# Gadersd/stable-diffusion-xl-burn

Hardware: NVIDIA H100
Metric: unet_sampler_steps_per_sec_1024x1024_bs1 (higher is better)
Workload: dtype f16

## Files before the change

### stable-diffusion-xl-burn_b200/csrc/attention.cu

```cuda
#include <stdlib.h>

#include "common.cuh"
#include "kernels.h"

namespace sdxl {

static constexpr int kTileBytes = 128 * 128;
static constexpr int kKvStages = 3;
static constexpr int kConsumerWarps = 8;
static constexpr int kAttnThreads = kConsumerWarps * 32 + 32;
static constexpr int kAttnSmem = 1024  + kTileBytes + 2 * kKvStages * kTileBytes + 256;

__device__ __forceinline__ float ex2_approx(float x) {
  float y;
  asm("ex2.approx.ftz.f32 %0, %1;" : "=f"(y) : "f"(x));
  return y;
}
__device__ __forceinline__ uint32_t pack_half2(float a, float b) {
  __half2 t = __floats2half2_rn(a, b);
  return *reinterpret_cast<uint32_t*>(&t);
}

__device__ __forceinline__ void attn_key_block(float (&o)[32], float (&m)[2], float (&l)[2], uint32_t q_addr, const uint8_t* sK,
                                               const uint8_t* sV, uint64_t* kv_full, uint64_t* kv_empty, int j, int kb, int S,
                                               float sl2e, int lane) {
  const int st = j % kKvStages;
  mbar_wait_nocall(&kv_full[st], (j / kKvStages) & 1);
  float s[64];
  wg_fence();
  const uint32_t k_addr = smem_u32(sK + st * kTileBytes);
#pragma unroll
  for (int k = 0; k < 4; ++k) wgmma_ss_n128(s, wg_desc_sw128(q_addr + 32 * k), wg_desc_sw128(k_addr + 32 * k), k);
  wg_commit();
  wg_wait<0>();
  if (kb * 128 + 128 > S) {
#pragma unroll
    for (int jj = 0; jj < 16; ++jj)
#pragma unroll
      for (int e = 0; e < 2; ++e)
        if (kb * 128 + 8 * jj + 2 * (lane & 3) + e >= S) { s[4 * jj + e] = -INFINITY; s[4 * jj + 2 + e] = -INFINITY; }
  }
  uint32_t pa[32];
#pragma unroll
  for (int h = 0; h < 2; ++h) {
    float mx = -INFINITY;
#pragma unroll
    for (int jj = 0; jj < 16; ++jj) mx = fmaxf(mx, fmaxf(s[4 * jj + 2 * h], s[4 * jj + 2 * h + 1]));
    mx = fmaxf(mx, __shfl_xor_sync(0xffffffffu, mx, 1));
    mx = fmaxf(mx, __shfl_xor_sync(0xffffffffu, mx, 2));
    const float m_new = fmaxf(m[h], mx);
    const float alpha = ex2_approx((m[h] - m_new) * sl2e);
    const float mb = m_new * sl2e;
    float sum = 0.f;
#pragma unroll
    for (int jj = 0; jj < 16; ++jj) {
      const float p0 = ex2_approx(fmaf(s[4 * jj + 2 * h], sl2e, -mb));
      const float p1 = ex2_approx(fmaf(s[4 * jj + 2 * h + 1], sl2e, -mb));
      sum += p0 + p1;
      pa[4 * (jj >> 1) + 2 * (jj & 1) + h] = pack_half2(p0, p1);
    }
    l[h] = l[h] * alpha + sum;
    m[h] = m_new;
#pragma unroll
    for (int jj = 0; jj < 8; ++jj) { o[4 * jj + 2 * h] *= alpha; o[4 * jj + 2 * h + 1] *= alpha; }
  }
  wg_fence();
  const uint32_t v_addr = smem_u32(sV + st * kTileBytes);
#pragma unroll
  for (int kk = 0; kk < 8; ++kk)
    wgmma_rs_n64_tb(o, *reinterpret_cast<const uint32_t(*)[4]>(pa + 4 * kk), wg_desc_sw128(v_addr + 2048 * kk));
  wg_commit();
  wg_wait<0>();
  if (lane == 0) mbar_arrive(&kv_empty[st]);
}

struct IpSrc {
  const CUtensorMap* tk;
  const CUtensorMap* tv;
  int S, k_col0, v_col0;
  const float* scale;
  const float* mask;
};
__device__ __forceinline__ IpSrc ip_source(const AttnParams& p, int k) {
  if (k == 0) return {&p.tmKip, &p.tmVip, p.S_ip, p.k_ip_col0, p.v_ip_col0, p.ip_scale, p.ip_mask};
  const AttnIpSource& s = p.ip_src[k - 1];
  return {&s.tm, &s.tm, s.S, s.k_col0, s.v_col0, s.scale, s.mask};
}

template <bool kIp>
__global__ void __launch_bounds__(kAttnThreads, 1) attention_kernel(const __grid_constant__ AttnParams p) {
  extern __shared__ uint8_t smem_raw[];
  uint8_t* smem = reinterpret_cast<uint8_t*>((reinterpret_cast<uintptr_t>(smem_raw) + 1023) & ~uintptr_t(1023));
  uint8_t* sQ = smem;
  uint8_t* sK = sQ + kTileBytes;
  uint8_t* sV = sK + kKvStages * kTileBytes;
  uint64_t* bars = reinterpret_cast<uint64_t*>(sV + kKvStages * kTileBytes);
  uint64_t* q_full = bars;
  uint64_t* kv_full = q_full + 1;
  uint64_t* kv_empty = kv_full + kKvStages;

  const int warp = threadIdx.x >> 5, lane = threadIdx.x & 31;
  const int nblk = (p.S + 127) / 128;
  const int nqt = (p.T + 127) / 128;
  const int qt = blockIdx.x % nqt, head = (blockIdx.x / nqt) % p.n_head, b = blockIdx.x / (nqt * p.n_head);

  if (threadIdx.x == 0) {
    tma_prefetch_desc(&p.tmQ);
    tma_prefetch_desc(&p.tmK);
    tma_prefetch_desc(&p.tmV);
    if constexpr (kIp) {
      tma_prefetch_desc(&p.tmKip);
      tma_prefetch_desc(&p.tmVip);
      for (int k = 1; k < p.n_src; ++k) tma_prefetch_desc(&p.ip_src[k - 1].tm);
    }
    mbar_init(q_full, 1);
    for (int i = 0; i < kKvStages; ++i) { mbar_init(&kv_full[i], 1); mbar_init(&kv_empty[i], kConsumerWarps); }
    fence_barrier_init();
  }
  __syncthreads();
  griddep_wait();
  griddep_launch_dependents();

  if (warp == kConsumerWarps) {
    if (lane != 0) return;
    mbar_expect_tx(q_full, kTileBytes);
    tma_load_3d(sQ, &p.tmQ, q_full, p.q_col0 + head * 64, qt * 128, b);
    for (int j = 0; j < nblk; ++j) {
      const int st = j % kKvStages;
      mbar_wait_nocall(&kv_empty[st], ((j / kKvStages) & 1) ^ 1);
      mbar_expect_tx(&kv_full[st], 2 * kTileBytes);
      tma_load_3d(sK + st * kTileBytes, &p.tmK, &kv_full[st], p.k_col0 + head * 64, j * 128, b);
      tma_load_3d(sV + st * kTileBytes, &p.tmV, &kv_full[st], p.v_col0 + head * 64, j * 128, b);
    }
    if constexpr (kIp) {
      int j = nblk;
      for (int k = 0; k < p.n_src; ++k) {
        const IpSrc s = ip_source(p, k);
        const int nb = (s.S + 127) / 128;
        for (int kb = 0; kb < nb; ++kb, ++j) {
          const int st = j % kKvStages;
          mbar_wait_nocall(&kv_empty[st], ((j / kKvStages) & 1) ^ 1);
          mbar_expect_tx(&kv_full[st], 2 * kTileBytes);
          tma_load_3d(sK + st * kTileBytes, s.tk, &kv_full[st], s.k_col0 + head * 64, kb * 128, b);
          tma_load_3d(sV + st * kTileBytes, s.tv, &kv_full[st], s.v_col0 + head * 64, kb * 128, b);
        }
      }
    }
    return;
  }

  const int wg = warp >> 2;
  const float sl2e = p.scale_log2e;
  const uint32_t q_addr = smem_u32(sQ) + (uint32_t)wg * (64 * 128);
  float o[32];
#pragma unroll
  for (int i = 0; i < 32; ++i) o[i] = 0.f;
  float m[2] = {-INFINITY, -INFINITY}, l[2] = {0.f, 0.f};
  mbar_wait_nocall(q_full, 0);
  for (int j = 0; j < nblk; ++j) {
    const int st = j % kKvStages;
    mbar_wait_nocall(&kv_full[st], (j / kKvStages) & 1);
    float s[64];
    wg_fence();
    const uint32_t k_addr = smem_u32(sK + st * kTileBytes);
#pragma unroll
    for (int k = 0; k < 4; ++k) wgmma_ss_n128(s, wg_desc_sw128(q_addr + 32 * k), wg_desc_sw128(k_addr + 32 * k), k);
    wg_commit();
    wg_wait<0>();
    if (j * 128 + 128 > p.S) {
#pragma unroll
      for (int jj = 0; jj < 16; ++jj)
#pragma unroll
        for (int e = 0; e < 2; ++e)
          if (j * 128 + 8 * jj + 2 * (lane & 3) + e >= p.S) { s[4 * jj + e] = -INFINITY; s[4 * jj + 2 + e] = -INFINITY; }
    }
    uint32_t pa[32];
#pragma unroll
    for (int h = 0; h < 2; ++h) {
      float mx = -INFINITY;
#pragma unroll
      for (int jj = 0; jj < 16; ++jj) mx = fmaxf(mx, fmaxf(s[4 * jj + 2 * h], s[4 * jj + 2 * h + 1]));
      mx = fmaxf(mx, __shfl_xor_sync(0xffffffffu, mx, 1));
      mx = fmaxf(mx, __shfl_xor_sync(0xffffffffu, mx, 2));
      const float m_new = fmaxf(m[h], mx);
      const float alpha = ex2_approx((m[h] - m_new) * sl2e);
      const float mb = m_new * sl2e;
      float sum = 0.f;
#pragma unroll
      for (int jj = 0; jj < 16; ++jj) {
        const float p0 = ex2_approx(fmaf(s[4 * jj + 2 * h], sl2e, -mb));
        const float p1 = ex2_approx(fmaf(s[4 * jj + 2 * h + 1], sl2e, -mb));
        sum += p0 + p1;
        pa[4 * (jj >> 1) + 2 * (jj & 1) + h] = pack_half2(p0, p1);
      }
      l[h] = l[h] * alpha + sum;
      m[h] = m_new;
#pragma unroll
      for (int jj = 0; jj < 8; ++jj) { o[4 * jj + 2 * h] *= alpha; o[4 * jj + 2 * h + 1] *= alpha; }
    }
    wg_fence();
    const uint32_t v_addr = smem_u32(sV + st * kTileBytes);
#pragma unroll
    for (int kk = 0; kk < 8; ++kk)
      wgmma_rs_n64_tb(o, *reinterpret_cast<const uint32_t(*)[4]>(pa + 4 * kk), wg_desc_sw128(v_addr + 2048 * kk));
    wg_commit();
    wg_wait<0>();
    if (lane == 0) mbar_arrive(&kv_empty[st]);
  }
  const int r = wg * 64 + (warp & 3) * 16 + (lane >> 2);
  if constexpr (kIp) {
    float acc[32];
#pragma unroll
    for (int h = 0; h < 2; ++h) {
      float lt = l[h];
      lt += __shfl_xor_sync(0xffffffffu, lt, 1);
      lt += __shfl_xor_sync(0xffffffffu, lt, 2);
      const float inv = 1.0f / lt;
#pragma unroll
      for (int jj = 0; jj < 8; ++jj) {
        acc[4 * jj + 2 * h] = o[4 * jj + 2 * h] * inv;
        acc[4 * jj + 2 * h + 1] = o[4 * jj + 2 * h + 1] * inv;
      }
    }
    int j = nblk;
    for (int k = 0; k < p.n_src; ++k) {
#pragma unroll
      for (int h = 0; h < 2; ++h) { m[h] = -INFINITY; l[h] = 0.f; }
#pragma unroll
      for (int i = 0; i < 32; ++i) o[i] = 0.f;
      const int S = ip_source(p, k).S;
      for (int kb = 0; kb * 128 < S; ++kb, ++j) attn_key_block(o, m, l, q_addr, sK, sV, kv_full, kv_empty, j, kb, S, sl2e, lane);
      const IpSrc s = ip_source(p, k);
      const float sk = *s.scale;
#pragma unroll
      for (int h = 0; h < 2; ++h) {
        float lt = l[h];
        lt += __shfl_xor_sync(0xffffffffu, lt, 1);
        lt += __shfl_xor_sync(0xffffffffu, lt, 2);
        const float inv = 1.0f / lt;
        const int t = qt * 128 + r + 8 * h;
        const float w = (s.mask && t < p.T) ? sk * s.mask[t] : sk;
#pragma unroll
        for (int jj = 0; jj < 8; ++jj) {
          acc[4 * jj + 2 * h] = fmaf(w, o[4 * jj + 2 * h] * inv, acc[4 * jj + 2 * h]);
          acc[4 * jj + 2 * h + 1] = fmaf(w, o[4 * jj + 2 * h + 1] * inv, acc[4 * jj + 2 * h + 1]);
        }
      }
    }
#pragma unroll
    for (int h = 0; h < 2; ++h) {
      const int t = qt * 128 + r + 8 * h;
      if (t < p.T) {
        __half* out = p.out + ((size_t)b * p.T + t) * p.ldo + head * 64 + 2 * (lane & 3);
#pragma unroll
        for (int jj = 0; jj < 8; ++jj)
          *reinterpret_cast<__half2*>(out + 8 * jj) = __floats2half2_rn(acc[4 * jj + 2 * h], acc[4 * jj + 2 * h + 1]);
      }
    }
  } else {
#pragma unroll
    for (int h = 0; h < 2; ++h) {
      float lt = l[h];
      lt += __shfl_xor_sync(0xffffffffu, lt, 1);
      lt += __shfl_xor_sync(0xffffffffu, lt, 2);
      const float inv = 1.0f / lt;
      const int t = qt * 128 + r + 8 * h;
      if (t < p.T) {
        __half* out = p.out + ((size_t)b * p.T + t) * p.ldo + head * 64 + 2 * (lane & 3);
#pragma unroll
        for (int jj = 0; jj < 8; ++jj)
          *reinterpret_cast<__half2*>(out + 8 * jj) = __floats2half2_rn(o[4 * jj + 2 * h] * inv, o[4 * jj + 2 * h + 1] * inv);
      }
    }
  }
}

__device__ __forceinline__ float cubic_w1(float x) { return ((-0.75f + 2.f) * x - (-0.75f + 3.f)) * x * x + 1.f; }
__device__ __forceinline__ float cubic_w2(float x) { return ((-0.75f * x - 5.f * -0.75f) * x + 8.f * -0.75f) * x - 4.f * -0.75f; }
__device__ __forceinline__ float cubic_1d(float x0, float x1, float x2, float x3, float t) {
  return x0 * cubic_w2(t + 1.f) + x1 * cubic_w1(t) + x2 * cubic_w1(1.f - t) + x3 * cubic_w2(2.f - t);
}
__global__ void ip_mask_resize_kernel(const float* __restrict__ mask, int H, int W, int mh, int mw, int T, float* __restrict__ out) {
  const int i = blockIdx.x * blockDim.x + threadIdx.x;
  if (i >= T) return;
  if (i >= mh * mw) { out[i] = 0.f; return; }
  const int oy = i / mw, ox = i % mw;
  const float ry = (float)H / mh * (oy + 0.5f) - 0.5f, rx = (float)W / mw * (ox + 0.5f) - 0.5f;
  const int iy = (int)floorf(ry), ix = (int)floorf(rx);
  const float ty = ry - iy, tx = rx - ix;
  float row[4];
#pragma unroll
  for (int k = 0; k < 4; ++k) {
    const float* m = mask + (size_t)min(max(iy - 1 + k, 0), H - 1) * W;
    row[k] = cubic_1d(m[min(max(ix - 1, 0), W - 1)], m[min(max(ix, 0), W - 1)], m[min(max(ix + 1, 0), W - 1)],
                      m[min(max(ix + 2, 0), W - 1)], tx);
  }
  out[i] = cubic_1d(row[0], row[1], row[2], row[3], ty);
}

int ip_mask_resize_launch(cudaStream_t st, const float* mask, int H, int W, int mh, int mw, int T, float* out) {
  if (H < 1 || W < 1 || mh < 1 || mw < 1 || T < 1) return 2002;
  ip_mask_resize_kernel<<<(T + 255) / 256, 256, 0, st>>>(mask, H, W, mh, mw, T, out);
  return (int)cudaGetLastError();
}

static bool g_attn_attr[2][64];
int attention_launch(cudaStream_t st, const AttnParams& p) {
  if (p.T < 1 || p.S < 1 || (p.ldo & 1)) return 2002;
  const bool ip = p.S_ip > 0;
  if (ip && (!p.ip_scale || p.n_src < 1 || p.n_src > ATTN_MAX_SRC)) return 2002;
  for (int k = 1; ip && k < p.n_src; ++k)
    if (p.ip_src[k - 1].S < 1 || !p.ip_src[k - 1].scale) return 2002;
  auto kernel = ip ? attention_kernel<true> : attention_kernel<false>;
  int r = smem_optin(kernel, kAttnSmem, g_attn_attr[ip]);
  if (r) return r;
  const long tiles = (long)p.B * p.n_head * ((p.T + 127) / 128);
  return launch_kernel(kernel, dim3((unsigned)tiles), dim3(kAttnThreads), (size_t)kAttnSmem, st, true, p);
}

}
```

### stable-diffusion-xl-burn_b200/csrc/kernels.h

```cpp
#pragma once
#include <cuda.h>
#include <cuda_fp16.h>
#include <cuda_runtime.h>
#include <stdint.h>

namespace sdxl {

bool pdl_enabled();
template <typename... KArgs, typename... Args>
inline int launch_kernel(void (*kernel)(KArgs...), dim3 grid, dim3 block, size_t smem, cudaStream_t st, bool pdl,
                         Args&&... args) {
  cudaLaunchConfig_t cfg{};
  cfg.gridDim = grid;
  cfg.blockDim = block;
  cfg.dynamicSmemBytes = smem;
  cfg.stream = st;
  cudaLaunchAttribute attr[1];
  attr[0].id = cudaLaunchAttributeProgrammaticStreamSerialization;
  attr[0].val.programmaticStreamSerializationAllowed = 1;
  cfg.attrs = attr;
  cfg.numAttrs = (pdl && pdl_enabled()) ? 1 : 0;
  return (int)cudaLaunchKernelEx(&cfg, kernel, static_cast<KArgs>(args)...);
}
template <typename... KArgs, typename... Args>
inline int launch_kernel_cluster(void (*kernel)(KArgs...), dim3 grid, dim3 block, size_t smem, cudaStream_t st, bool pdl,
                                 int cluster_size, Args&&... args) {
  cudaLaunchConfig_t cfg{};
  cfg.gridDim = grid;
  cfg.blockDim = block;
  cfg.dynamicSmemBytes = smem;
  cfg.stream = st;
  cudaLaunchAttribute attr[2];
  int n = 0;
  if (cluster_size > 1) {
    attr[n].id = cudaLaunchAttributeClusterDimension;
    attr[n].val.clusterDim.x = cluster_size;
    attr[n].val.clusterDim.y = 1;
    attr[n].val.clusterDim.z = 1;
    ++n;
  }
  if (pdl && pdl_enabled()) {
    attr[n].id = cudaLaunchAttributeProgrammaticStreamSerialization;
    attr[n].val.programmaticStreamSerializationAllowed = 1;
    ++n;
  }
  cfg.attrs = attr;
  cfg.numAttrs = n;
  return (int)cudaLaunchKernelEx(&cfg, kernel, static_cast<KArgs>(args)...);
}

template <typename K>
inline int smem_optin(K kernel, int bytes, bool (&done)[64]) {
  int dev = 0;
  cudaError_t e = cudaGetDevice(&dev);
  if (e != cudaSuccess) return (int)e;
  if (dev < 0 || dev >= 64) return 2001;
  if (!done[dev]) {
    e = cudaFuncSetAttribute(kernel, cudaFuncAttributeMaxDynamicSharedMemorySize, bytes);
    if (e != cudaSuccess) return (int)e;
    done[dev] = true;
  }
  return 0;
}

constexpr int IGEMM_MAX_SEG = 20;
struct IgemmSeg {
  int16_t map;
  int16_t dw, dh;
  int16_t db;
  int32_t nkb;
};
enum IgemmMode : int { IGEMM_LINEAR = 0, IGEMM_GEGLU = 1 };
struct alignas(64) IgemmParams {
  CUtensorMap tmA0, tmA1, tmB;
  IgemmSeg seg[IGEMM_MAX_SEG];
  int nseg;
  int Wt, Ht, Bt;
  int W, H, Bn;
  int tilesW, tilesH, tilesB, tilesN;
  int N;
  int BN;
  int nstages;
  int mode;
  void* out;
  int out_f32;
  int ldo;
  const float* bias;
  int bias_bstride;
  const float* res;
  int ldr;
  int opix_row, opix_w, opix_off;
};
int make_tmap_act(CUtensorMap* tm, const __half* base, int Bn, int H, int W, int C, int pitch, int Wt,
                  int Ht, int Bt);
int make_tmap_wgt(CUtensorMap* tm, const __half* base, int N, int K, int BN);
void igemm_pick_box(int W, int H, int* Wt, int* Ht, int* Bt);
struct IgemmOperands {
  const __half* a0; int a0Bn, a0H, a0W, a0C, a0pitch;
  const __half* a1; int a1Bn, a1H, a1W, a1C, a1pitch;
  const __half* w; int N, Ktot;
};
int igemm_configure(IgemmParams& p, const IgemmOperands& o, int outW, int outH, int outB, int mode, int geglu_bn);
int igemm_launch(cudaStream_t st, IgemmParams& p);
int igemm_pick_bn(int m_tiles, int N, int num_sms, bool geglu);

constexpr int ATTN_MAX_SRC = 8;
struct AttnIpSource {
  CUtensorMap tm;
  int S, k_col0, v_col0;
  const float* scale;
  const float* mask;
};
struct AttnParams {
  CUtensorMap tmQ, tmK, tmV;
  int T, S, n_head, B;
  int q_col0, k_col0, v_col0;
  __half* out;
  int ldo;
  float scale_log2e;
  CUtensorMap tmKip, tmVip;
  int S_ip;
  int k_ip_col0, v_ip_col0;
  const float* ip_scale;
  int n_src;
  const float* ip_mask;
  AttnIpSource ip_src[ATTN_MAX_SRC - 1];
};
int make_tmap_rows(CUtensorMap* tm, const __half* base, int rows_per_batch, int nbatch, int cols, int pitch);
int attention_launch(cudaStream_t st, const AttnParams& p);
int ip_mask_resize_launch(cudaStream_t st, const float* mask, int H, int W, int mh, int mw, int T, float* out);

struct GnParams {
  const float* x1; int C1;
  const float* x2; int C2;
  int B, HW, n_group;
  const float* gamma; const float* beta;
  float eps;
  int silu;
  __half* y;
  __half* raw;
  float* partial;
  int nchunk;
  __half* y_lo;
};
size_t gn_scratch_floats(int B, int n_group);
int gn_scratch_init(cudaStream_t st, float* scratch, int B, int n_group);
int gn_launch(cudaStream_t st, GnParams& p);
int layernorm_launch(cudaStream_t st, const float* x, const float* gamma, const float* beta, float eps,
                     int rows, int C, __half* y);

int gemv_launch(cudaStream_t st, const float* in, int in_bstride, int Bv, int K, const __half* W, int ldw,
                const float* bias, const float* add, int add_bstride, int N, int in_silu, int out_silu,
                float* out, int out_bstride);
int timestep_embedding_launch(cudaStream_t st, const int* t_dev, int nt, int dim, float max_period,
                              float* out);
int conv_in_launch(cudaStream_t st, const __half* x, int B, int Cin, int H, int W, const float* w,
                   const float* bias, int Cout, float* y);
int conv_in_launch_t(cudaStream_t st, const void* x, int x_f32, int Bx, int B, int Cin, int H, int W,
                     const float* w, const float* bias, int Cout, float* y, const float* add = nullptr, int n_add = 1);
int conv_in_cat_launch(cudaStream_t st, const void* x, int x_f32, int Bx, int B, int C1, const float* x2, int n2, int C2, int H, int W,
                       const float* w, const float* bias, int Cout, float* y, const float* add = nullptr, int n_add = 1);
int silu_f16_launch(cudaStream_t st, const float* x, int B, int H, int W, int C, int phase, __half* y);
int scale_weights_launch(cudaStream_t st, const __half* w, size_t nw, const float* b, int nb, float s, __half* wo, float* bo);
int upsample2x_launch(cudaStream_t st, const float* x, int B, int H, int W, int C, __half* y);
int phase_split_launch(cudaStream_t st, const float* x, int B, int H, int W, int C, __half* y);
int cast_f32_to_f16_launch(cudaStream_t st, const float* x, size_t n, __half* y);
int cast_f16_to_f32_launch(cudaStream_t st, const __half* x, size_t n, float* y);
int nhwc_to_nchw_f16_launch(cudaStream_t st, const float* x, int B, int HW, int C, int ldx, __half* y);
int nhwc_to_nchw_f32_launch(cudaStream_t st, const float* x, int B, int HW, int C, int ldx, float* y);
int cfg_ddim_launch(cudaStream_t st, const float* eps, int ld, int Bimg, int C, int HW, int use_cfg,
                    float guidance, float sqrt_a, float sqrt_1ma, float sqrt_ap, float sqrt_1map,
                    float* x, __half* x16);
int cfg_pag_ddim_launch(cudaStream_t st, const float* eps, int ld, int Bimg, int C, int HW, int use_cfg, float guidance, float p_t,
                        float sqrt_a, float sqrt_1ma, float sqrt_ap, float sqrt_1map, float* x);
int pag_identity_launch(cudaStream_t st, const __half* qkv, int C, long rows, __half* out);
int inpaint_blend_launch(cudaStream_t st, float* x, const float* ref, const float* noise,
                         const uint8_t* mask, size_t n_per_img_batch, int nfwd, float sqrt_a,
                         float sqrt_1ma, __half* x16);
int axpby_launch(cudaStream_t st, float* x, const float* noise, size_t n, float sa, float sb);
int randn_launch(cudaStream_t st, float* out, size_t n, uint64_t seed, uint64_t subseq);
int dup_latent_f16_launch(cudaStream_t st, const float* x, size_t n, int nfwd, __half* x16);

int softmax_rows_launch(cudaStream_t st, const float* S, size_t lds, int rows, int cols, float scale, __half* P,
                        size_t ldp);
int transpose_f16_launch(cudaStream_t st, const __half* x, size_t ldx, int rows, int cols, __half* y, size_t ldy);
int post_quant_launch(cudaStream_t st, const float* x, int B, int C, int HW, const float* w, const float* bias,
                      float inv_scale, float* y);
int image_u8_launch(cudaStream_t st, const float* x, long npix, int ldx, uint8_t* out);

int image_from_u8_launch(cudaStream_t st, const uint8_t* in, int B, long HW, float* out);
int quant_out_launch(cudaStream_t st, const float* x, int B, int Cz, int Cout, long HW, const float* w, const float* bias,
                     float scale, float* y);

int embed_tokens_launch(cudaStream_t st, const int* tokens, int rows, int T, int C, int n_vocab, const __half* tok_emb,
                        const __half* pos_emb, float* x, int* err);
int attention_small_launch(cudaStream_t st, const __half* q, int q_pitch, int q_col0, const __half* k, const __half* v,
                           int kv_pitch, int k_col0, int v_col0, int B, int T, int S, int n_head, const __half* mask,
                           int causal, __half* out, int ldo, int head_dim = 64);
int patchify_launch(cudaStream_t st, const float* pixels, int N, int S, int p, int Kpad, __half* y);
int vision_embed_ln_launch(cudaStream_t st, const float* patches, const __half* cls, const __half* pos, int N, int T, int C,
                           const float* gamma, const float* beta, float eps, float* x);
int mlp_act_launch(cudaStream_t st, const float* x, size_t n, int quick, __half* y);
int ln_gather_f32_launch(cudaStream_t st, const float* x, const int* idx, int B, int T, int C, const float* gamma,
                         const float* beta, float eps, float* y);
int perceiver_ln_launch(cudaStream_t st, const float* x, const float* lat, int n, int L, int Q, int C, const float* g1,
                        const float* b1, const float* g2, const float* b2, float eps, __half* kv, __half* q);

int pixel_unshuffle_launch(cudaStream_t st, const float* x, int n, int C, int H, int W, __half* y);
int relu_f16_launch(cudaStream_t st, const float* x, size_t n, __half* y);
int avg_pool2_f16_launch(cudaStream_t st, const float* x, int n, int H, int W, int C, __half* y);
int t2i_add_launch(cudaStream_t st, float* x, const float* F, long per_img, int B, int n_hint, const int* t, const int* t_min);

int transpose_linear_launch(cudaStream_t st, const __half* src, int K, int N, __half* dst, int Kpad,
                            int dst_row0, int geglu_bn);
int repack_conv_launch(cudaStream_t st, const __half* src, int O, int I, int KH, int KW, __half* dst,
                       int Ktot, int col0, int Ipad);
int repack_upconv_launch(cudaStream_t st, const __half* src, int O, int I, __half* dst, int Ipad);
int vec_add_f32_launch(cudaStream_t st, float* dst, const float* src, int n);
int bias_to_f32_launch(cudaStream_t st, const __half* src, int N, float* dst, int geglu_bn, int accumulate);

#define LORA_MAX_TERMS 16
struct LoraTerm { const __half* up; const __half* down; int r; float coef; };
struct LoraMergeParams {
  int N, Kd, taps;
  int nterm;
  LoraTerm term[LORA_MAX_TERMS];
  const void* src; void* dst; int f32;
  size_t ld; int row0, col0, Ipad, geglu_bn;
  float* delta_out;
};
int lora_merge_launch(cudaStream_t st, const LoraMergeParams& p);
int lora_upconv_merge_launch(cudaStream_t st, const __half* src, const float* delta, int O, int I, __half* dst, int Ipad);

}
```

### stable-diffusion-xl-burn_b200/csrc/testing.cu

```cuda
#include "kernels.h"

#define SDXL_TEST_API extern "C" __attribute__((visibility("default")))

using namespace sdxl;

SDXL_TEST_API int sdxl_test_igemm(void* stream, const void* a0, int a0Bn, int a0H, int a0W, int a0C, int a0pitch, const void* a1,
                                  int a1Bn, int a1H, int a1W, int a1C, int a1pitch, const void* w, int N, int Ktot, int outW,
                                  int outH, int outB, int mode, int geglu_bn, const int* segs, int nseg, void* out, int out_f32,
                                  int ldo, const float* bias, int bias_bstride, const float* res, int ldr, int opix_row,
                                  int opix_w, int opix_off) {
  if (nseg < 1 || nseg > IGEMM_MAX_SEG) return 5002;
  IgemmParams p{};
  p.nseg = nseg;
  for (int i = 0; i < nseg; ++i)
    p.seg[i] = {(int16_t)segs[5 * i], (int16_t)segs[5 * i + 1], (int16_t)segs[5 * i + 2], (int16_t)segs[5 * i + 3], segs[5 * i + 4]};
  p.out = out; p.out_f32 = out_f32; p.ldo = ldo;
  p.bias = bias; p.bias_bstride = bias_bstride;
  p.res = res; p.ldr = ldr;
  const IgemmOperands o{(const __half*)a0, a0Bn, a0H, a0W, a0C, a0pitch, (const __half*)a1, a1Bn, a1H, a1W, a1C, a1pitch,
                        (const __half*)w, N, Ktot};
  if (int r = igemm_configure(p, o, outW, outH, outB, mode, geglu_bn)) return r;
  if (opix_row) { p.opix_row = opix_row; p.opix_w = opix_w; p.opix_off = opix_off; }
  return igemm_launch((cudaStream_t)stream, p);
}

SDXL_TEST_API int sdxl_test_attention(void* stream, const void* q, int q_pitch, int q_col0, const void* kv, int kv_pitch, int k_col0,
                                      int v_col0, int B, int T, int S, int n_head, void* out, int ldo, const void* kip,
                                      int kip_pitch, int k_ip_col0, int v_ip_col0, int S_ip, const float* ip_scale) {
  AttnParams p{};
  p.T = T; p.S = S; p.n_head = n_head; p.B = B;
  p.q_col0 = q_col0; p.k_col0 = k_col0; p.v_col0 = v_col0;
  p.out = (__half*)out; p.ldo = ldo;
  p.scale_log2e = (float)(1.4426950408889634 / 8.0);
  int r = make_tmap_rows(&p.tmQ, (const __half*)q, T, B, q_pitch, q_pitch);
  if (!r) r = make_tmap_rows(&p.tmK, (const __half*)kv, S, B, kv_pitch, kv_pitch);
  if (r) return r;
  p.tmV = p.tmK;
  if (kip) {
    p.S_ip = S_ip; p.k_ip_col0 = k_ip_col0; p.v_ip_col0 = v_ip_col0; p.ip_scale = ip_scale; p.n_src = 1;
    if ((r = make_tmap_rows(&p.tmKip, (const __half*)kip, S_ip, B, kip_pitch, kip_pitch))) return r;
    p.tmVip = p.tmKip;
  }
  return attention_launch((cudaStream_t)stream, p);
}

SDXL_TEST_API int sdxl_test_attention_multi(void* stream, const void* q, int q_pitch, int q_col0, const void* kv, int kv_pitch, int k_col0,
                                            int v_col0, int B, int T, int S, int n_head, void* out, int ldo, int n_src,
                                            const void* const* src_kv, const int* src_info, const float* const* scales,
                                            const float* const* masks) {
  if (n_src < 1 || n_src > ATTN_MAX_SRC) return 5003;
  AttnParams p{};
  p.T = T; p.S = S; p.n_head = n_head; p.B = B;
  p.q_col0 = q_col0; p.k_col0 = k_col0; p.v_col0 = v_col0;
  p.out = (__half*)out; p.ldo = ldo;
  p.scale_log2e = (float)(1.4426950408889634 / 8.0);
  int r = make_tmap_rows(&p.tmQ, (const __half*)q, T, B, q_pitch, q_pitch);
  if (!r) r = make_tmap_rows(&p.tmK, (const __half*)kv, S, B, kv_pitch, kv_pitch);
  if (r) return r;
  p.tmV = p.tmK;
  p.n_src = n_src;
  for (int k = 0; k < n_src; ++k) {
    const int* f = src_info + 4 * k;
    CUtensorMap tm;
    if ((r = make_tmap_rows(&tm, (const __half*)src_kv[k], f[3], B, f[0], f[0]))) return r;
    if (k == 0) {
      p.tmKip = p.tmVip = tm;
      p.S_ip = f[3]; p.k_ip_col0 = f[1]; p.v_ip_col0 = f[2]; p.ip_scale = scales[0]; p.ip_mask = masks[0];
    } else {
      p.ip_src[k - 1] = {tm, f[3], f[1], f[2], scales[k], masks[k]};
    }
  }
  return attention_launch((cudaStream_t)stream, p);
}

SDXL_TEST_API int sdxl_test_ip_mask_resize(void* stream, const float* mask, int H, int W, int mh, int mw, int T, float* out) {
  return ip_mask_resize_launch((cudaStream_t)stream, mask, H, W, mh, mw, T, out);
}

SDXL_TEST_API int sdxl_test_attention_small(void* stream, const void* q, int q_pitch, int q_col0, const void* k, const void* v,
                                            int kv_pitch, int k_col0, int v_col0, int B, int T, int S, int n_head, const void* mask,
                                            int causal, void* out, int ldo, int head_dim) {
  return attention_small_launch((cudaStream_t)stream, (const __half*)q, q_pitch, q_col0, (const __half*)k, (const __half*)v, kv_pitch,
                                k_col0, v_col0, B, T, S, n_head, (const __half*)mask, causal, (__half*)out, ldo, head_dim);
}

SDXL_TEST_API int sdxl_test_perceiver_ln(void* stream, const float* x, const float* lat, int n, int L, int Q, int C, const float* g1,
                                         const float* b1, const float* g2, const float* b2, float eps, void* kv, void* q) {
  return perceiver_ln_launch((cudaStream_t)stream, x, lat, n, L, Q, C, g1, b1, g2, b2, eps, (__half*)kv, (__half*)q);
}

SDXL_TEST_API size_t sdxl_test_gn_scratch_floats(int B, int n_group) { return gn_scratch_floats(B, n_group); }
SDXL_TEST_API int sdxl_test_gn_scratch_init(void* stream, float* scratch, int B, int n_group) {
  return gn_scratch_init((cudaStream_t)stream, scratch, B, n_group);
}
SDXL_TEST_API int sdxl_test_gn(void* stream, const float* x1, int C1, const float* x2, int C2, int B, int HW, int n_group,
                               const float* gamma, const float* beta, float eps, int silu, void* y, void* raw, void* y_lo,
                               float* scratch) {
  GnParams p{x1, C1, x2, C2, B, HW, n_group, gamma, beta, eps, silu, (__half*)y, (__half*)raw, scratch, 0, (__half*)y_lo};
  return gn_launch((cudaStream_t)stream, p);
}

SDXL_TEST_API int sdxl_test_gemv(void* stream, const float* in, int in_bstride, int Bv, int K, const void* W, int ldw,
                                 const float* bias, const float* add, int add_bstride, int N, int in_silu, int out_silu, float* out,
                                 int out_bstride) {
  return gemv_launch((cudaStream_t)stream, in, in_bstride, Bv, K, (const __half*)W, ldw, bias, add, add_bstride, N, in_silu, out_silu,
                     out, out_bstride);
}

SDXL_TEST_API int sdxl_test_conv_in(void* stream, const void* x, int x_f32, int Bx, int B, int Cin, int H, int W, const float* w,
                                    const float* bias, int Cout, float* y, const float* add, int n_add) {
  return conv_in_launch_t((cudaStream_t)stream, x, x_f32, Bx, B, Cin, H, W, w, bias, Cout, y, add, n_add);
}
SDXL_TEST_API int sdxl_test_conv_in_cat(void* stream, const void* x, int x_f32, int Bx, int B, int C1, const float* x2, int n2, int C2,
                                        int H, int W, const float* w, const float* bias, int Cout, float* y) {
  return conv_in_cat_launch((cudaStream_t)stream, x, x_f32, Bx, B, C1, x2, n2, C2, H, W, w, bias, Cout, y);
}

SDXL_TEST_API int sdxl_test_pag_identity(void* stream, const void* qkv, int C, long rows, void* out) {
  return pag_identity_launch((cudaStream_t)stream, (const __half*)qkv, C, rows, (__half*)out);
}
SDXL_TEST_API int sdxl_test_cfg_pag_ddim(void* stream, const float* eps, int ld, int Bimg, int C, int HW, int use_cfg, float guidance,
                                         float p_t, float sqrt_a, float sqrt_1ma, float sqrt_ap, float sqrt_1map, float* x) {
  return cfg_pag_ddim_launch((cudaStream_t)stream, eps, ld, Bimg, C, HW, use_cfg, guidance, p_t, sqrt_a, sqrt_1ma, sqrt_ap, sqrt_1map, x);
}

SDXL_TEST_API int sdxl_test_repack_upconv(void* stream, const void* src, int O, int I, void* dst, int Ipad) {
  return repack_upconv_launch((cudaStream_t)stream, (const __half*)src, O, I, (__half*)dst, Ipad);
}
SDXL_TEST_API int sdxl_test_repack_conv(void* stream, const void* src, int O, int I, int KH, int KW, void* dst, int Ktot, int col0,
                                        int Ipad) {
  return repack_conv_launch((cudaStream_t)stream, (const __half*)src, O, I, KH, KW, (__half*)dst, Ktot, col0, Ipad);
}
SDXL_TEST_API int sdxl_test_transpose_linear(void* stream, const void* src, int K, int N, void* dst, int Kpad, int dst_row0,
                                             int geglu_bn) {
  return transpose_linear_launch((cudaStream_t)stream, (const __half*)src, K, N, (__half*)dst, Kpad, dst_row0, geglu_bn);
}
SDXL_TEST_API int sdxl_test_bias_to_f32(void* stream, const void* src, int N, float* dst, int geglu_bn, int accumulate) {
  return bias_to_f32_launch((cudaStream_t)stream, (const __half*)src, N, dst, geglu_bn, accumulate);
}

SDXL_TEST_API int sdxl_test_lora_merge(void* stream, int N, int Kd, int taps, int nterm, const void* const* up, const void* const* down,
                                       const int* r, const float* coef, const void* src, void* dst, int f32, size_t ld, int row0,
                                       int col0, int Ipad, int geglu_bn, float* delta_out) {
  if (nterm < 1 || nterm > LORA_MAX_TERMS) return 1;
  LoraMergeParams p{};
  p.N = N; p.Kd = Kd; p.taps = taps; p.nterm = nterm;
  for (int i = 0; i < nterm; ++i) p.term[i] = {(const __half*)up[i], (const __half*)down[i], r[i], coef[i]};
  p.src = src; p.dst = dst; p.f32 = f32;
  p.ld = ld; p.row0 = row0; p.col0 = col0; p.Ipad = Ipad; p.geglu_bn = geglu_bn;
  p.delta_out = delta_out;
  return lora_merge_launch((cudaStream_t)stream, p);
}
SDXL_TEST_API int sdxl_test_lora_upconv_merge(void* stream, const void* src, const float* delta, int O, int I, void* dst, int Ipad) {
  return lora_upconv_merge_launch((cudaStream_t)stream, (const __half*)src, delta, O, I, (__half*)dst, Ipad);
}
```

### stable-diffusion-xl-burn_b200/sdxl_b200/_testing.py

```python
from __future__ import annotations

import ctypes as C
import os
from typing import Optional, Sequence

import torch

from ._lib import SdxlError, SdxlLibraryMissing

HERE = os.path.dirname(os.path.abspath(__file__))
LIB_PATH = os.path.join(HERE, "libsdxl_b200_testing.so")

P, I, F = C.c_void_p, C.c_int, C.c_float
PROTOTYPES = {
    "sdxl_test_igemm": (I, [P, P, I, I, I, I, I, P, I, I, I, I, I, P, I, I, I, I, I, I, I, P, I, P, I, I, P, I, P, I, I, I, I]),
    "sdxl_test_attention": (I, [P, P, I, I, P, I, I, I, I, I, I, I, P, I, P, I, I, I, I, P]),
    "sdxl_test_attention_multi": (I, [P, P, I, I, P, I, I, I, I, I, I, I, P, I, I, P, P, P, P]),
    "sdxl_test_ip_mask_resize": (I, [P, P, I, I, I, I, I, P]),
    "sdxl_test_attention_small": (I, [P, P, I, I, P, P, I, I, I, I, I, I, I, P, I, P, I, I]),
    "sdxl_test_perceiver_ln": (I, [P, P, P, I, I, I, I, P, P, P, P, F, P, P]),
    "sdxl_test_gn_scratch_floats": (C.c_size_t, [I, I]),
    "sdxl_test_gn_scratch_init": (I, [P, P, I, I]),
    "sdxl_test_gn": (I, [P, P, I, P, I, I, I, I, P, P, F, I, P, P, P, P]),
    "sdxl_test_gemv": (I, [P, P, I, I, I, P, I, P, P, I, I, I, I, P, I]),
    "sdxl_test_conv_in": (I, [P, P, I, I, I, I, I, I, P, P, I, P, P, I]),
    "sdxl_test_conv_in_cat": (I, [P, P, I, I, I, I, P, I, I, I, I, P, P, I, P]),
    "sdxl_test_pag_identity": (I, [P, P, I, C.c_long, P]),
    "sdxl_test_cfg_pag_ddim": (I, [P, P, I, I, I, I, I, F, F, F, F, F, F, P]),
    "sdxl_test_repack_upconv": (I, [P, P, I, I, P, I]),
    "sdxl_test_repack_conv": (I, [P, P, I, I, I, I, P, I, I, I]),
    "sdxl_test_transpose_linear": (I, [P, P, I, I, P, I, I, I]),
    "sdxl_test_bias_to_f32": (I, [P, P, I, P, I, I]),
    "sdxl_test_lora_merge": (I, [P, I, I, I, I, P, P, P, P, P, P, I, C.c_size_t, I, I, I, I, P]),
    "sdxl_test_lora_upconv_merge": (I, [P, P, P, I, I, P, I]),
}
_lib = None


def load() -> C.CDLL:
    global _lib
    if _lib is None:
        if not os.path.exists(LIB_PATH):
            raise SdxlLibraryMissing(f"{LIB_PATH} not found: build it with `python stable-diffusion-xl-burn_b200/build.py`")
        lib = C.CDLL(LIB_PATH)
        for name, (res, args) in PROTOTYPES.items():
            fn = getattr(lib, name)
            fn.restype = res
            fn.argtypes = args
        _lib = lib
    return _lib


def _p(t: Optional[torch.Tensor]):
    if t is None:
        return None
    assert t.is_cuda and t.is_contiguous(), "kernel operands are contiguous CUDA tensors"
    return t.data_ptr()


def _call(name: str, *args) -> None:
    lib = load()
    rc = getattr(lib, name)(torch.cuda.current_stream().cuda_stream, *args)
    if rc != 0:
        raise SdxlError(f"{name} failed ({rc})")


def igemm(a0: torch.Tensor, a0_shape: Sequence[int], w: torch.Tensor, N: int, Ktot: int, out_whb: Sequence[int],
          segs: Sequence[Sequence[int]], out: torch.Tensor, ldo: int, *, a1: Optional[torch.Tensor] = None,
          a1_shape: Sequence[int] = (0, 0, 0, 0), bias: Optional[torch.Tensor] = None, bias_bstride: int = 0,
          res: Optional[torch.Tensor] = None, ldr: int = 0, mode: int = 0, geglu_bn: int = 0,
          opix: Optional[Sequence[int]] = None) -> None:
    seg = (C.c_int * (5 * len(segs)))(*[int(v) for s in segs for v in s])
    o = opix or (0, 0, 0)
    _call("sdxl_test_igemm", _p(a0), *a0_shape, a0_shape[3], _p(a1), *a1_shape, a1_shape[3], _p(w), N, Ktot, *out_whb, mode,
          geglu_bn, seg, len(segs), _p(out), int(out.dtype == torch.float32), ldo, _p(bias), bias_bstride, _p(res), ldr, *o)


def attention(q: torch.Tensor, q_pitch: int, q_col0: int, kv: torch.Tensor, kv_pitch: int, k_col0: int, v_col0: int,
              B: int, T: int, S: int, n_head: int, out: torch.Tensor, ldo: int, kip: Optional[torch.Tensor] = None,
              kip_pitch: int = 0, k_ip_col0: int = 0, v_ip_col0: int = 0, S_ip: int = 0,
              ip_scale: Optional[torch.Tensor] = None) -> None:
    _call("sdxl_test_attention", _p(q), q_pitch, q_col0, _p(kv), kv_pitch, k_col0, v_col0, B, T, S, n_head, _p(out), ldo,
          _p(kip), kip_pitch, k_ip_col0, v_ip_col0, S_ip, _p(ip_scale))


def attention_multi(q: torch.Tensor, q_pitch: int, q_col0: int, kv: torch.Tensor, kv_pitch: int, k_col0: int, v_col0: int,
                    B: int, T: int, S: int, n_head: int, out: torch.Tensor, ldo: int, sources: Sequence[tuple]) -> None:
    n = len(sources)
    kvs = (C.c_void_p * n)(*[_p(s[0]) for s in sources])
    info = (C.c_int * (4 * n))(*[int(v) for s in sources for v in (s[1], s[2], s[3], s[4])])
    scales = (C.c_void_p * n)(*[_p(s[5]) for s in sources])
    masks = (C.c_void_p * n)(*[_p(s[6]) for s in sources])
    _call("sdxl_test_attention_multi", _p(q), q_pitch, q_col0, _p(kv), kv_pitch, k_col0, v_col0, B, T, S, n_head, _p(out), ldo, n,
          kvs, info, scales, masks)


def ip_mask_resize(mask: torch.Tensor, mh: int, mw: int, T: int) -> torch.Tensor:
    out = torch.empty(T, device=mask.device, dtype=torch.float32)
    _call("sdxl_test_ip_mask_resize", _p(mask), mask.shape[0], mask.shape[1], mh, mw, T, _p(out))
    return out


def attention_small(q, q_pitch, q_col0, k, v, kv_pitch, k_col0, v_col0, B, T, S, n_head, mask, causal, out, ldo,
                    head_dim) -> None:
    _call("sdxl_test_attention_small", _p(q), q_pitch, q_col0, _p(k), _p(v), kv_pitch, k_col0, v_col0, B, T, S, n_head,
          _p(mask), int(causal), _p(out), ldo, head_dim)


def perceiver_ln(x, lat, n, L, Q, C, g1, b1, g2, b2, eps, kv, q) -> None:
    _call("sdxl_test_perceiver_ln", _p(x), _p(lat), n, L, Q, C, _p(g1), _p(b1), _p(g2), _p(b2), eps, _p(kv), _p(q))


def gn_scratch(B: int, n_group: int) -> torch.Tensor:
    s = torch.empty(load().sdxl_test_gn_scratch_floats(B, n_group), dtype=torch.float32, device="cuda")
    _call("sdxl_test_gn_scratch_init", _p(s), B, n_group)
    return s


def group_norm(x1, x2, B, HW, n_group, gamma, beta, eps, silu, y, raw, y_lo, scratch) -> None:
    C1 = x1.shape[-1]
    C2 = 0 if x2 is None else x2.shape[-1]
    _call("sdxl_test_gn", _p(x1), C1, _p(x2), C2, B, HW, n_group, _p(gamma), _p(beta), eps, int(silu), _p(y), _p(raw),
          _p(y_lo), _p(scratch))


def gemv(inp, in_bstride, Bv, K, W, ldw, bias, add, add_bstride, N, in_silu, out_silu, out, out_bstride) -> None:
    _call("sdxl_test_gemv", _p(inp), in_bstride, Bv, K, _p(W), ldw, _p(bias), _p(add), add_bstride, N, int(in_silu),
          int(out_silu), _p(out), out_bstride)


def conv_in(x, Bx, B, Cin, H, W, w, bias, Cout, y, add=None, n_add=1) -> None:
    _call("sdxl_test_conv_in", _p(x), int(x.dtype == torch.float32), Bx, B, Cin, H, W, _p(w), _p(bias), Cout, _p(y), _p(add),
          n_add)


def conv_in_cat(x, Bx, B, C1, x2, n2, C2, H, W, w, bias, Cout, y) -> None:
    _call("sdxl_test_conv_in_cat", _p(x), int(x.dtype == torch.float32), Bx, B, C1, _p(x2), n2, C2, H, W, _p(w), _p(bias), Cout, _p(y))


def pag_identity(qkv: torch.Tensor, C: int, rows: int, out: torch.Tensor) -> None:
    _call("sdxl_test_pag_identity", _p(qkv), C, rows, _p(out))


def cfg_pag_ddim(eps, ld, Bimg, C, HW, use_cfg, guidance, p_t, sqrt_a, sqrt_1ma, sqrt_ap, sqrt_1map, x) -> None:
    _call("sdxl_test_cfg_pag_ddim", _p(eps), ld, Bimg, C, HW, int(use_cfg), guidance, p_t, sqrt_a, sqrt_1ma, sqrt_ap, sqrt_1map, _p(x))


def repack_upconv(src, O, I, dst, Ipad) -> None:
    _call("sdxl_test_repack_upconv", _p(src), O, I, _p(dst), Ipad)


def repack_conv(src, O, I, KH, KW, dst, Ktot, col0, Ipad) -> None:
    _call("sdxl_test_repack_conv", _p(src), O, I, KH, KW, _p(dst), Ktot, col0, Ipad)


def transpose_linear(src, K, N, dst, Kpad, dst_row0=0, geglu_bn=0) -> None:
    _call("sdxl_test_transpose_linear", _p(src), K, N, _p(dst), Kpad, dst_row0, geglu_bn)


def bias_to_f32(src, N, dst, geglu_bn=0, accumulate=False) -> None:
    _call("sdxl_test_bias_to_f32", _p(src), N, _p(dst), geglu_bn, int(accumulate))


def lora_merge(N, Kd, taps, terms, src, dst, ld, row0=0, col0=0, Ipad=0, geglu_bn=0, delta_out=None) -> None:
    n = len(terms)
    ups = (C.c_void_p * n)(*[_p(u) for u, _, _ in terms])
    downs = (C.c_void_p * n)(*[_p(d) for _, d, _ in terms])
    rs = (C.c_int * n)(*[u.shape[1] for u, _, _ in terms])
    coefs = (C.c_float * n)(*[float(c) for _, _, c in terms])
    _call("sdxl_test_lora_merge", N, Kd, taps, n, ups, downs, rs, coefs, _p(src), _p(dst), int(dst.dtype == torch.float32), ld,
          row0, col0, Ipad, geglu_bn, _p(delta_out))


def lora_upconv_merge(src, delta, O, I, dst, Ipad) -> None:
    _call("sdxl_test_lora_upconv_merge", _p(src), _p(delta), O, I, _p(dst), Ipad)
```

Measured before the change: 27.65.

## Overlap next QK wgmma with PV in attention and skip unneeded rescale

Splits the attention key block into a QK issue step and a softmax/PV step, then issues the next block's QK wgmma before waiting on the current PV wgmma. This lets the tensor-core work of consecutive blocks overlap. It also skips rescaling the output accumulator when no row maximum grew in the warp. A polynomial exp2 emulation is added to offload work from the MUFU unit, but its column fraction is set to zero, so only the test kernel uses it for now. The s register array is now live across iterations, which raises register pressure.

```diff
diff --git a/stable-diffusion-xl-burn_b200/csrc/attention.cu b/stable-diffusion-xl-burn_b200/csrc/attention.cu
--- a/stable-diffusion-xl-burn_b200/csrc/attention.cu
+++ b/stable-diffusion-xl-burn_b200/csrc/attention.cu
@@ -16,22 +16,38 @@
   asm("ex2.approx.ftz.f32 %0, %1;" : "=f"(y) : "f"(x));
   return y;
 }
+__device__ __forceinline__ float ex2_poly(float x) {
+  x = fmaxf(x, -127.f);
+  const float t = x + 12582912.f;
+  const float f = x - (t - 12582912.f);
+  float p = fmaf(9.58323106e-3f, f, 5.59063852e-2f);
+  p = fmaf(p, f, 2.40240902e-1f);
+  p = fmaf(p, f, 6.93124235e-1f);
+  p = fmaf(p, f, 1.f);
+  return __int_as_float(__float_as_int(p) + (__float_as_int(t) << 23));
+}
+static constexpr int kPolyExp2 = 0;
+__device__ constexpr bool poly_col(int jj) { return jj * (kPolyExp2 / 4) / 16 != (jj + 1) * (kPolyExp2 / 4) / 16; }
 __device__ __forceinline__ uint32_t pack_half2(float a, float b) {
   __half2 t = __floats2half2_rn(a, b);
   return *reinterpret_cast<uint32_t*>(&t);
 }
 
-__device__ __forceinline__ void attn_key_block(float (&o)[32], float (&m)[2], float (&l)[2], uint32_t q_addr, const uint8_t* sK,
-                                               const uint8_t* sV, uint64_t* kv_full, uint64_t* kv_empty, int j, int kb, int S,
-                                               float sl2e, int lane) {
+__device__ __forceinline__ void attn_qk(float (&s)[64], uint32_t q_addr, const uint8_t* sK, uint64_t* kv_full, int j) {
   const int st = j % kKvStages;
   mbar_wait_nocall(&kv_full[st], (j / kKvStages) & 1);
-  float s[64];
   wg_fence();
   const uint32_t k_addr = smem_u32(sK + st * kTileBytes);
 #pragma unroll
   for (int k = 0; k < 4; ++k) wgmma_ss_n128(s, wg_desc_sw128(q_addr + 32 * k), wg_desc_sw128(k_addr + 32 * k), k);
   wg_commit();
+}
+
+template <bool kNext>
+__device__ __forceinline__ void attn_key_block(float (&s)[64], float (&o)[32], float (&m)[2], float (&l)[2], uint32_t q_addr,
+                                               const uint8_t* sK, const uint8_t* sV, uint64_t* kv_full, uint64_t* kv_empty, int j,
+                                               int kb, int S, float sl2e, int lane) {
+  const int st = j % kKvStages;
   wg_wait<0>();
   if (kb * 128 + 128 > S) {
 #pragma unroll
@@ -40,7 +56,7 @@
       for (int e = 0; e < 2; ++e)
         if (kb * 128 + 8 * jj + 2 * (lane & 3) + e >= S) { s[4 * jj + e] = -INFINITY; s[4 * jj + 2 + e] = -INFINITY; }
   }
-  uint32_t pa[32];
+  float m_new[2];
 #pragma unroll
   for (int h = 0; h < 2; ++h) {
     float mx = -INFINITY;
@@ -48,21 +64,31 @@
     for (int jj = 0; jj < 16; ++jj) mx = fmaxf(mx, fmaxf(s[4 * jj + 2 * h], s[4 * jj + 2 * h + 1]));
     mx = fmaxf(mx, __shfl_xor_sync(0xffffffffu, mx, 1));
     mx = fmaxf(mx, __shfl_xor_sync(0xffffffffu, mx, 2));
-    const float m_new = fmaxf(m[h], mx);
-    const float alpha = ex2_approx((m[h] - m_new) * sl2e);
-    const float mb = m_new * sl2e;
+    m_new[h] = fmaxf(m[h], mx);
+  }
+  const bool grown = __any_sync(0xffffffffu, m_new[0] != m[0] || m_new[1] != m[1]);
+  uint32_t pa[32];
+#pragma unroll
+  for (int h = 0; h < 2; ++h) {
+    const float mb = m_new[h] * sl2e;
     float sum = 0.f;
 #pragma unroll
     for (int jj = 0; jj < 16; ++jj) {
-      const float p0 = ex2_approx(fmaf(s[4 * jj + 2 * h], sl2e, -mb));
-      const float p1 = ex2_approx(fmaf(s[4 * jj + 2 * h + 1], sl2e, -mb));
+      const float x0 = fmaf(s[4 * jj + 2 * h], sl2e, -mb), x1 = fmaf(s[4 * jj + 2 * h + 1], sl2e, -mb);
+      const float p0 = poly_col(jj) ? ex2_poly(x0) : ex2_approx(x0);
+      const float p1 = poly_col(jj) ? ex2_poly(x1) : ex2_approx(x1);
       sum += p0 + p1;
       pa[4 * (jj >> 1) + 2 * (jj & 1) + h] = pack_half2(p0, p1);
     }
-    l[h] = l[h] * alpha + sum;
-    m[h] = m_new;
-#pragma unroll
-    for (int jj = 0; jj < 8; ++jj) { o[4 * jj + 2 * h] *= alpha; o[4 * jj + 2 * h + 1] *= alpha; }
+    if (grown) {
+      const float alpha = ex2_approx((m[h] - m_new[h]) * sl2e);
+      l[h] = fmaf(l[h], alpha, sum);
+#pragma unroll
+      for (int jj = 0; jj < 8; ++jj) { o[4 * jj + 2 * h] *= alpha; o[4 * jj + 2 * h + 1] *= alpha; }
+    } else {
+      l[h] += sum;
+    }
+    m[h] = m_new[h];
   }
   wg_fence();
   const uint32_t v_addr = smem_u32(sV + st * kTileBytes);
@@ -70,7 +96,12 @@
   for (int kk = 0; kk < 8; ++kk)
     wgmma_rs_n64_tb(o, *reinterpret_cast<const uint32_t(*)[4]>(pa + 4 * kk), wg_desc_sw128(v_addr + 2048 * kk));
   wg_commit();
-  wg_wait<0>();
+  if constexpr (kNext) {
+    attn_qk(s, q_addr, sK, kv_full, j + 1);
+    wg_wait<1>();
+  } else {
+    wg_wait<0>();
+  }
   if (lane == 0) mbar_arrive(&kv_empty[st]);
 }
 
@@ -157,56 +188,10 @@
   for (int i = 0; i < 32; ++i) o[i] = 0.f;
   float m[2] = {-INFINITY, -INFINITY}, l[2] = {0.f, 0.f};
   mbar_wait_nocall(q_full, 0);
-  for (int j = 0; j < nblk; ++j) {
-    const int st = j % kKvStages;
-    mbar_wait_nocall(&kv_full[st], (j / kKvStages) & 1);
-    float s[64];
-    wg_fence();
-    const uint32_t k_addr = smem_u32(sK + st * kTileBytes);
-#pragma unroll
-    for (int k = 0; k < 4; ++k) wgmma_ss_n128(s, wg_desc_sw128(q_addr + 32 * k), wg_desc_sw128(k_addr + 32 * k), k);
-    wg_commit();
-    wg_wait<0>();
-    if (j * 128 + 128 > p.S) {
-#pragma unroll
-      for (int jj = 0; jj < 16; ++jj)
-#pragma unroll
-        for (int e = 0; e < 2; ++e)
-          if (j * 128 + 8 * jj + 2 * (lane & 3) + e >= p.S) { s[4 * jj + e] = -INFINITY; s[4 * jj + 2 + e] = -INFINITY; }
-    }
-    uint32_t pa[32];
-#pragma unroll
-    for (int h = 0; h < 2; ++h) {
-      float mx = -INFINITY;
-#pragma unroll
-      for (int jj = 0; jj < 16; ++jj) mx = fmaxf(mx, fmaxf(s[4 * jj + 2 * h], s[4 * jj + 2 * h + 1]));
-      mx = fmaxf(mx, __shfl_xor_sync(0xffffffffu, mx, 1));
-      mx = fmaxf(mx, __shfl_xor_sync(0xffffffffu, mx, 2));
-      const float m_new = fmaxf(m[h], mx);
-      const float alpha = ex2_approx((m[h] - m_new) * sl2e);
-      const float mb = m_new * sl2e;
-      float sum = 0.f;
-#pragma unroll
-      for (int jj = 0; jj < 16; ++jj) {
-        const float p0 = ex2_approx(fmaf(s[4 * jj + 2 * h], sl2e, -mb));
-        const float p1 = ex2_approx(fmaf(s[4 * jj + 2 * h + 1], sl2e, -mb));
-        sum += p0 + p1;
-        pa[4 * (jj >> 1) + 2 * (jj & 1) + h] = pack_half2(p0, p1);
-      }
-      l[h] = l[h] * alpha + sum;
-      m[h] = m_new;
-#pragma unroll
-      for (int jj = 0; jj < 8; ++jj) { o[4 * jj + 2 * h] *= alpha; o[4 * jj + 2 * h + 1] *= alpha; }
-    }
-    wg_fence();
-    const uint32_t v_addr = smem_u32(sV + st * kTileBytes);
-#pragma unroll
-    for (int kk = 0; kk < 8; ++kk)
-      wgmma_rs_n64_tb(o, *reinterpret_cast<const uint32_t(*)[4]>(pa + 4 * kk), wg_desc_sw128(v_addr + 2048 * kk));
-    wg_commit();
-    wg_wait<0>();
-    if (lane == 0) mbar_arrive(&kv_empty[st]);
-  }
+  float s[64];
+  attn_qk(s, q_addr, sK, kv_full, 0);
+  for (int j = 0; j + 1 < nblk; ++j) attn_key_block<true>(s, o, m, l, q_addr, sK, sV, kv_full, kv_empty, j, j, p.S, sl2e, lane);
+  attn_key_block<false>(s, o, m, l, q_addr, sK, sV, kv_full, kv_empty, nblk - 1, nblk - 1, p.S, sl2e, lane);
   const int r = wg * 64 + (warp & 3) * 16 + (lane >> 2);
   if constexpr (kIp) {
     float acc[32];
@@ -229,7 +214,10 @@
 #pragma unroll
       for (int i = 0; i < 32; ++i) o[i] = 0.f;
       const int S = ip_source(p, k).S;
-      for (int kb = 0; kb * 128 < S; ++kb, ++j) attn_key_block(o, m, l, q_addr, sK, sV, kv_full, kv_empty, j, kb, S, sl2e, lane);
+      for (int kb = 0; kb * 128 < S; ++kb, ++j) {
+        attn_qk(s, q_addr, sK, kv_full, j);
+        attn_key_block<false>(s, o, m, l, q_addr, sK, sV, kv_full, kv_empty, j, kb, S, sl2e, lane);
+      }
       const IpSrc s = ip_source(p, k);
       const float sk = *s.scale;
 #pragma unroll
@@ -318,4 +306,14 @@
   return launch_kernel(kernel, dim3((unsigned)tiles), dim3(kAttnThreads), (size_t)kAttnSmem, st, true, p);
 }
 
-}
+__global__ void ex2_poly_kernel(const float* __restrict__ x, float* __restrict__ y, int n) {
+  const int i = blockIdx.x * blockDim.x + threadIdx.x;
+  if (i < n) y[i] = ex2_poly(x[i]);
+}
+int ex2_poly_launch(cudaStream_t st, const float* x, float* y, int n) {
+  if (n < 1) return 2002;
+  ex2_poly_kernel<<<(n + 255) / 256, 256, 0, st>>>(x, y, n);
+  return (int)cudaGetLastError();
+}
+
+}
diff --git a/stable-diffusion-xl-burn_b200/csrc/kernels.h b/stable-diffusion-xl-burn_b200/csrc/kernels.h
--- a/stable-diffusion-xl-burn_b200/csrc/kernels.h
+++ b/stable-diffusion-xl-burn_b200/csrc/kernels.h
@@ -128,6 +128,7 @@
 };
 int make_tmap_rows(CUtensorMap* tm, const __half* base, int rows_per_batch, int nbatch, int cols, int pitch);
 int attention_launch(cudaStream_t st, const AttnParams& p);
+int ex2_poly_launch(cudaStream_t st, const float* x, float* y, int n);
 int ip_mask_resize_launch(cudaStream_t st, const float* mask, int H, int W, int mh, int mw, int T, float* out);
 
 struct GnParams {
diff --git a/stable-diffusion-xl-burn_b200/csrc/testing.cu b/stable-diffusion-xl-burn_b200/csrc/testing.cu
--- a/stable-diffusion-xl-burn_b200/csrc/testing.cu
+++ b/stable-diffusion-xl-burn_b200/csrc/testing.cu
@@ -71,6 +71,10 @@
     }
   }
   return attention_launch((cudaStream_t)stream, p);
+}
+
+SDXL_TEST_API int sdxl_test_ex2_poly(void* stream, const float* x, float* y, int n) {
+  return ex2_poly_launch((cudaStream_t)stream, x, y, n);
 }
 
 SDXL_TEST_API int sdxl_test_ip_mask_resize(void* stream, const float* mask, int H, int W, int mh, int mw, int T, float* out) {
diff --git a/stable-diffusion-xl-burn_b200/sdxl_b200/_testing.py b/stable-diffusion-xl-burn_b200/sdxl_b200/_testing.py
--- a/stable-diffusion-xl-burn_b200/sdxl_b200/_testing.py
+++ b/stable-diffusion-xl-burn_b200/sdxl_b200/_testing.py
@@ -16,6 +16,7 @@
     "sdxl_test_igemm": (I, [P, P, I, I, I, I, I, P, I, I, I, I, I, P, I, I, I, I, I, I, I, P, I, P, I, I, P, I, P, I, I, I, I]),
     "sdxl_test_attention": (I, [P, P, I, I, P, I, I, I, I, I, I, I, P, I, P, I, I, I, I, P]),
     "sdxl_test_attention_multi": (I, [P, P, I, I, P, I, I, I, I, I, I, I, P, I, I, P, P, P, P]),
+    "sdxl_test_ex2_poly": (I, [P, P, P, I]),
     "sdxl_test_ip_mask_resize": (I, [P, P, I, I, I, I, I, P]),
     "sdxl_test_attention_small": (I, [P, P, I, I, P, P, I, I, I, I, I, I, I, P, I, P, I, I]),
     "sdxl_test_perceiver_ln": (I, [P, P, P, I, I, I, I, P, P, P, P, F, P, P]),
@@ -93,6 +94,12 @@
     masks = (C.c_void_p * n)(*[_p(s[6]) for s in sources])
     _call("sdxl_test_attention_multi", _p(q), q_pitch, q_col0, _p(kv), kv_pitch, k_col0, v_col0, B, T, S, n_head, _p(out), ldo, n,
           kvs, info, scales, masks)
+
+
+def ex2_poly(x: torch.Tensor) -> torch.Tensor:
+    y = torch.empty_like(x)
+    _call("sdxl_test_ex2_poly", _p(x), _p(y), x.numel())
+    return y
 
 
 def ip_mask_resize(mask: torch.Tensor, mh: int, mw: int, T: int) -> torch.Tensor:
```

Result: no change. 27.67, median of 6 (+0.1%).
